# beenotung/bpe-tokenizer

Hardware: NVIDIA B200
Metric: mergeUntil merges/sec (higher is better)
Workload: dtype u32

## Files before the change

### bpe_tokenizer_b200/build.py

```python
from __future__ import annotations

import os
import shutil
import subprocess
import sys

HERE = os.path.dirname(os.path.abspath(__file__))
CSRC = os.path.join(HERE, "csrc")
LIB = os.path.join(HERE, "libbpe_b200.so")
SOURCES = ["bpe_b200.cu", "synth.cpp"]
DEPS = ["common.cuh", "train_kernels.cuh", "encode_kernels.cuh", "encode_lanes.cuh", "encode_dp.cuh", "mg_kernels.cuh", "round_kernels.cuh", "text_kernels.cuh", os.path.join("..", "..", "include", "bpe_b200.h")]
NVCC_FLAGS = [
    "-gencode", "arch=compute_100a,code=sm_100a",
    "-lineinfo", "-O3", "-std=c++17", "-shared",
    "-Xcompiler", "-fPIC,-pthread",
]


def nvcc_path() -> str:
    for cand in (os.environ.get("NVCC"), shutil.which("nvcc"), "/usr/local/cuda/bin/nvcc"):
        if cand and os.path.exists(cand):
            return cand
    raise RuntimeError("nvcc not found")


def needs_build() -> bool:
    if not os.path.exists(LIB):
        return True
    t = os.path.getmtime(LIB)
    return any(os.path.getmtime(os.path.join(CSRC, f)) > t for f in SOURCES + DEPS)


def build(force: bool = False, verbose: bool = False, out: str = LIB) -> str:
    if not force and out == LIB and not needs_build():
        return LIB
    extra = ["-DBPE_FINE_PROF"] if os.environ.get("BPE_FINE_PROF") else []
    if os.environ.get("BPE_ML_THREADS"):
        extra.append("-DBPE_ML_THREADS=" + os.environ["BPE_ML_THREADS"])
    if os.environ.get("BPE_TBL_STRIDE"):
        extra.append("-DBPE_TBL_STRIDE=" + os.environ["BPE_TBL_STRIDE"])
    for knob in ("BPE_R_SMALL_LOG", "BPE_R_BATCH_LOG", "BPE_K1B_CHUNK_LOG"):
        if os.environ.get(knob):
            extra.append("-D%s=%s" % (knob, os.environ[knob]))
    if os.environ.get("BPE_RD_THREADS"):
        extra.append("-DBPE_RD_THREADS=" + os.environ["BPE_RD_THREADS"])
    cmd = [nvcc_path()] + NVCC_FLAGS + extra + (["-Xptxas", "-v"] if verbose else []) + ["-o", out] + [os.path.join(CSRC, f) for f in SOURCES]
    r = subprocess.run(cmd, capture_output=True, text=True)
    if verbose or r.returncode != 0:
        sys.stderr.write(r.stdout + r.stderr)
    if r.returncode != 0:
        raise RuntimeError("nvcc failed (%d)" % r.returncode)
    return out


SYNTH_LIB = os.path.join(HERE, "libbpe_synth.so")


def build_synth(force: bool = False) -> str:
    src = os.path.join(CSRC, "synth.cpp")
    if not force and os.path.exists(SYNTH_LIB) and os.path.getmtime(SYNTH_LIB) >= os.path.getmtime(src):
        return SYNTH_LIB
    cxx = os.environ.get("CXX") or shutil.which("g++") or "g++"
    r = subprocess.run([cxx, "-O2", "-std=c++17", "-shared", "-fPIC", "-pthread", "-o", SYNTH_LIB, src], capture_output=True, text=True)
    if r.returncode != 0:
        sys.stderr.write(r.stdout + r.stderr)
        raise RuntimeError("g++ failed on synth.cpp (%d)" % r.returncode)
    return SYNTH_LIB


if __name__ == "__main__":
    build_synth(force="--force" in sys.argv)
    print(build(force="--force" in sys.argv, verbose="-v" in sys.argv))
```

### bpe_tokenizer_b200/csrc/bpe_b200.cu

```cuda
#include "../../include/bpe_b200.h"

#include <algorithm>
#include <cstdarg>
#include <cstdio>
#include <cstdlib>
#include <chrono>
#include <cstring>
#include <functional>
#include <string>
#include <unordered_map>
#include <vector>

#include "encode_kernels.cuh"
#include "encode_lanes.cuh"
#include "encode_dp.cuh"
#include "train_kernels.cuh"
#include "mg_kernels.cuh"
#include "round_kernels.cuh"
#include "text_kernels.cuh"

using namespace bpe;

namespace {

// ... 934 lines not shown
  if (total > 0) {
    CK(cudaMemsetAsync(&e->d_st.p->err, 0, sizeof(uint32_t), e->stream));
    int blocks = (int)std::min<int64_t>((total / 4 + 255) / 256 + 1, (int64_t)e->grid(8));
    if (reinterpret_cast<const uint32_t*>(dev_ids + base_in) == e->slots.p + e->n_slots)
      k_validate_ids<<<blocks, 256, 0, e->stream>>>(e->slots.p + e->n_slots, (uint64_t)total, (uint32_t)e->n_tokens, &e->d_st.p->err);
    else
      k_ingest_ids<<<blocks, 256, 0, e->stream>>>(dev_ids + base_in, e->slots.p + e->n_slots, (uint64_t)total, (uint32_t)e->n_tokens, &e->d_st.p->err);
    CKL();
    CK(e->stage_off.reserve((size_t)n_docs + 1, 0, e->stream, 1.5));
    CK(cudaMemcpyAsync(e->stage_off.p, host_off, (size_t)(n_docs + 1) * sizeof(int64_t), cudaMemcpyHostToDevice, e->stream));
    int blocks2 = (int)std::min<int64_t>((n_docs + 255) / 256, (int64_t)e->grid(8));
    k_mark_docstarts<<<blocks2, 256, 0, e->stream>>>(e->slots.p, e->stage_off.p, n_docs, (int64_t)e->n_slots - base_in);
    CKL();
    uint32_t bad = 0;
    CK(cudaMemcpyAsync(&bad, &e->d_st.p->err, sizeof bad, cudaMemcpyDeviceToHost, e->stream));
    CK(cudaStreamSynchronize(e->stream));
    if (bad) {
      CK(cudaMemsetAsync(&e->d_st.p->err, 0, sizeof(uint32_t), e->stream));
      return fail(e, BPE_E_INVALID, "document holds a token index >= n_tokens (%d); call bpe_set_tokens first", e->n_tokens);
    }
  }
  for (int64_t d = 0; d < n_docs; d++) e->doc_off.push_back((int64_t)e->n_slots + (host_off[d + 1] - base_in));
  e->n_slots = new_n;
  e->live_tokens += (uint64_t)total;
  e->index_valid = false;
  e->hot_valid = false;
  return BPE_OK;
}


int ensure_round_buffers(bpe_engine* e) {
  if (!e->round_blocks) {
    int per_sm = 0;
    CK(cudaOccupancyMaxActiveBlocksPerMultiprocessor(&per_sm, k_merge_rounds, RD_THREADS, 0));
    if (per_sm < 1) return fail(e, BPE_E_CUDA, "k_merge_rounds does not fit on an SM");
    const int most = std::min({e->sm_count * per_sm, (int)(R_QCAP / RT), RD_THREADS / RT});
    e->round_blocks = std::min(e->sm_count, most);
    if (const char* v = getenv("BPE_LOOP_BLOCKS")) e->round_blocks = std::max(1, std::min(atoi(v), most));
  }
  const size_t cells = (size_t)2 * RB * 2 * ND_STRIDE;
  if (!e->r_cells.p) {
    CK(e->r_cells.reserve(cells));
    CK(cudaMemsetAsync(e->r_cells.p, 0, cells * 8, e->stream));
    CK(e->r_slotrows.reserve(cells));
    CK(e->r_lists.reserve((size_t)2 * e->round_blocks * R_LISTCAP));
    CK(e->r_bsites.reserve((size_t)2 * RB * R_SMALL));
    CK(e->r_state.reserve(1));
    CK(cudaMemsetAsync(e->r_state.p, 0, sizeof(RoundState), e->stream));
  }
  if (e->mg_world > 1 && !e->r_gcells.p) {
    CK(e->r_gcells.reserve(cells));
    CK(cudaMemsetAsync(e->r_gcells.p, 0, cells * 8, e->stream));
    CK(e->r_glists.reserve((size_t)2 * e->round_blocks * R_LISTCAP));
  }
  CK(e->r_gp.reserve((size_t)RT * e->round_blocks));
  CK(e->r_gk.reserve((size_t)RT * e->round_blocks));
  return BPE_OK;
}

RoundArgs round_args(bpe_engine* e, const LoopArgs& L, int round_k) {
  RoundArgs RA{};
  RA.L = L;
  RA.cells = e->r_cells.p;
  RA.slotrows = e->r_slotrows.p;
  RA.lists = e->r_lists.p;
  RA.bsites = e->r_bsites.p;
  RA.gp = e->r_gp.p;
  RA.gk = e->r_gk.p;
  RA.rs = e->r_state.p;
  RA.kmax = (uint32_t)round_k;
  RA.bar_mode = 1;
  if (const char* v = getenv("BPE_LOOP_BAR")) RA.bar_mode = atoi(v) ? 1 : 0;
  RA.mg_on = 0;
  RA.gcells = e->r_gcells.p;
  RA.glists = e->r_glists.p;
  return RA;
}

void round_stats(bpe_engine* e, const RoundState& hrs) {
  e->stats.loop_rounds = (int64_t)hrs.rounds;
  e->stats.loop_round_merges = (int64_t)hrs.round_merges;
  e->stats.loop_round_tried = (int64_t)hrs.tried;
  e->stats.loop_rounds_cut = (int64_t)hrs.rounds_cut_born;
}

int merge_until_device(bpe_engine* e, int64_t min_weight, int32_t max_length, int64_t max_iterations, bpe_merge* log,
                       int64_t log_cap, int64_t* n_done, const int32_t* dev_replay = nullptr) {
  *n_done = 0;
  CK(cudaSetDevice(e->device));
  if (e->n_slots == 0) return BPE_OK;
  TRY(ensure_index(e));
  uint32_t ml = max_length > 0 ? (uint32_t)max_length : 0;
  int64_t mw = min_weight > 0 ? min_weight : 2;
  if (!e->loop_blocks) {
    int per_sm = 0;
    CK(cudaOccupancyMaxActiveBlocksPerMultiprocessor(&per_sm, k_merge_loop, ML_THREADS, 0));
    if (per_sm < 1) return fail(e, BPE_E_CUDA, "k_merge_loop does not fit on an SM");
    int want = 1;
    if (const char* v = getenv("BPE_LOOP_PER_SM")) want = std::max(1, atoi(v));
    e->loop_blocks = e->sm_count * std::min(per_sm, want);
    if (const char* v = getenv("BPE_LOOP_BLOCKS")) e->loop_blocks = std::max(1, std::min(atoi(v), e->sm_count * per_sm));
  }
  bool use_rounds = !dev_replay;
// ... 57 lines not shown
    L.tbl_cap = e->tbl_cap;
    L.sites2 = e->sites2.p;
    L.A.sites_cap = (uint32_t)std::min<size_t>(L.A.sites_cap, e->sites2.cap);
    {
      int a = 12, b = 10, c = 2, ns = 256;
      if (const char* v = getenv("BPE_LOOP_P1_SITES")) a = atoi(v);
      if (const char* v = getenv("BPE_LOOP_P2_NEW")) b = atoi(v);
      if (const char* v = getenv("BPE_LOOP_P2_RW")) c = atoi(v);
      if (const char* v = getenv("BPE_LOOP_BAR_NS")) ns = atoi(v);
      if (a < 1 || a > 15) a = 12;
      if (b < 1 || c < 1 || b + c > 15) b = 10, c = 2;
      L.p1_sites = (uint32_t)a;
      L.p2_new = (uint32_t)b;
      L.p2_rw = (uint32_t)c;
      L.bar_ns = (uint32_t)std::max(32, std::min(ns, 4096));
    }
    const char* pf = getenv("BPE_LOOP_PREFETCH");
    L.prefetch = pf ? std::max(0, std::min(atoi(pf), 2)) : (use_rounds ? 0 : 1);
    L.replay = dev_replay ? dev_replay + 2 * done : nullptr;
    if (dev_replay) e->hot_valid = false;
    static const bool trace = getenv("BPE_TRACE") != nullptr;
    auto tw0 = std::chrono::steady_clock::now();
    k_loop_prepare<<<1, 32, 0, e->stream>>>(e->d_st.p, (uint32_t)e->n_tokens, e->barrier.p);
    e->stats.kernel_launches++;
    if (use_rounds && legacy_above) {
      L.min_weight = (uint32_t)std::max<int64_t>(mw, (int64_t)R_HUGE + 1);
      void* args[] = {&L};
      ce = cudaLaunchCooperativeKernel((void*)k_merge_loop, dim3(e->loop_blocks), dim3(ML_THREADS), args, 0, e->stream);
    } else if (use_rounds) {
      RoundArgs RA = round_args(e, L, round_k);
      k_rounds_prepare<<<1, 32, 0, e->stream>>>(e->r_state.p);
      e->stats.kernel_launches++;
      void* rargs[] = {&RA};
      ce = cudaLaunchCooperativeKernel((void*)k_merge_rounds, dim3(e->round_blocks), dim3(RD_THREADS), rargs, 0, e->stream);
    } else {
      void* args[] = {&L};
      ce = cudaLaunchCooperativeKernel((void*)k_merge_loop, dim3(e->loop_blocks), dim3(ML_THREADS), args, 0, e->stream);
    }
    if (ce != cudaSuccess) {
      rc = fail(e, BPE_E_CUDA, "cooperative launch of the mergeUntil kernel: %s", cudaGetErrorString(ce));
      break;
    }
    e->stats.kernel_launches++;
    if ((rc = fetch_state(e)) != BPE_OK) break;
    uint32_t iters = e->h_st->iters_done;
    if (trace) {
      double ms = std::chrono::duration<double, std::milli>(std::chrono::steady_clock::now() - tw0).count();
      fprintf(stderr, "[bpe] k_merge_loop: %u merges in %.2f ms, status %u, best_cnt %u, hot_n %u thresh %u, keys %u/%u\n", iters, ms,
              e->h_st->status, e->h_st->best_cnt, e->h_st->hot_n, e->h_st->hot_thresh, e->h_st->n_keys, e->tbl_cap);
    }
    if (iters) {
      tmp.resize(iters);
      ce = cudaMemcpyAsync(tmp.data(), e->dev_log.p, (size_t)iters * sizeof(MergeRec), cudaMemcpyDeviceToHost, e->stream);
      if (ce == cudaSuccess) ce = cudaStreamSynchronize(e->stream);
      if (ce != cudaSuccess) {
        rc = fail(e, BPE_E_CUDA, "merge log read-back: %s", cudaGetErrorString(ce));
        break;
      }
      for (uint32_t i = 0; i < iters; i++) {
        const MergeRec& r = tmp[i];
        log[done].a = r.a;
        log[done].b = r.b;
        log[done].c = r.c;
        log[done].reserved = 0;
        log[done].weight = r.weight;
        done++;
        e->h_len16.push_back(e->h_len16[r.a] + e->h_len16[r.b]);
// ... 209 lines not shown
    L.hot = e->hot.p;
    L.hot_cap = (uint32_t)std::min<size_t>(e->hot.cap, 0xFFFFFFF0u);
    L.hot_limit = e->hot_limit;
    L.cands = e->cands.p;
    L.cand_cap = (uint32_t)std::min<size_t>(e->cands.cap, 0xFFFFFFF0u);
    L.partials = e->partials.p;
    L.barrier = e->barrier.p;
    L.log = e->dev_log.p;
    L.log_cap = chunk;
    L.max_length = ml;
    L.min_weight = (uint32_t)std::min<int64_t>(mw, 0xFFFFFFFFll);
    L.max_tokens = BPE_MAX_TOKENS;
    L.tbl_cap = e->tbl_cap;
    L.replay = nullptr;
    P.M = mg_args(e);
    static const bool trace = getenv("BPE_TRACE") != nullptr;
    auto tw0 = std::chrono::steady_clock::now();
    k_loop_prepare<<<1, 32, 0, e->stream>>>(e->d_st.p, (uint32_t)e->n_tokens, e->barrier.p);
    e->stats.kernel_launches++;
    if (use_rounds && !legacy_above) {
      L.sites2 = e->sites2.p;
      L.A.sites_cap = (uint32_t)std::min<size_t>(L.A.sites_cap, e->sites2.cap);
      L.p1_sites = 12;
      L.p2_new = 10;
      L.p2_rw = 2;
      L.bar_ns = 256;
      L.prefetch = 0;
      RoundArgs RA = round_args(e, L, round_k);
      RA.mg_on = 1;
      RA.mg = P.M;
      k_rounds_prepare<<<1, 32, 0, e->stream>>>(e->r_state.p);
      e->stats.kernel_launches++;
      void* rargs[] = {&RA};
      ce = cudaLaunchCooperativeKernel((void*)k_merge_rounds, dim3(e->round_blocks), dim3(RD_THREADS), rargs, 0, e->stream);
    } else {
      if (use_rounds) L.min_weight = (uint32_t)std::max<int64_t>(mw, (int64_t)R_HUGE + 1);
      void* args[] = {&P};
      ce = cudaLaunchCooperativeKernel((void*)k_merge_loop_mg, dim3(e->mg_loop_blocks), dim3(ML_THREADS), args, 0, e->stream);
    }
    if (ce != cudaSuccess) {
      rc = fail(e, BPE_E_CUDA, "cooperative launch of the sharded mergeUntil kernel: %s", cudaGetErrorString(ce));
      break;
    }
    e->stats.kernel_launches++;
    if ((rc = fetch_state(e)) != BPE_OK) break;
    host_ms[2] += since(tw0);
    e->mg_epoch = e->h_st->mg_epoch;
    e->mg_tie_epoch = e->h_st->mg_tie_epoch;
    uint32_t iters = e->h_st->iters_done;
    if (trace) {
      double ms = std::chrono::duration<double, std::milli>(std::chrono::steady_clock::now() - tw0).count();
      fprintf(stderr, "[bpe r%d] k_merge_loop_mg: %u merges in %.2f ms, status %u, best_cnt %u, hot_n %u thresh %u, keys %u/%u err 0x%x gerr 0x%x\n",
              e->mg_rank, iters, ms, e->h_st->status, e->h_st->best_cnt, e->h_st->hot_n, e->h_st->hot_thresh, e->h_st->n_keys, e->tbl_cap,
              e->h_st->err, e->h_st->g_vals[0]);
    }
    auto tl = clk();
    if (iters) {
      tmp.resize(iters);
      ce = cudaMemcpyAsync(tmp.data(), e->dev_log.p, (size_t)iters * sizeof(MergeRec), cudaMemcpyDeviceToHost, e->stream);
      if (ce == cudaSuccess) ce = cudaStreamSynchronize(e->stream);
      if (ce != cudaSuccess) {
        rc = fail(e, BPE_E_CUDA, "merge log read-back: %s", cudaGetErrorString(ce));
        break;
      }
      for (uint32_t i = 0; i < iters; i++) {
        const MergeRec& r = tmp[i];
        log[done].a = r.a;
// ... 1216 lines not shown
```

### bpe_tokenizer_b200/csrc/round_kernels.cuh

```cuda
#pragma once
#include "train_kernels.cuh"
#include "mg_kernels.cuh"

namespace bpe {

#ifndef BPE_RD_THREADS
#define BPE_RD_THREADS 512
#endif
constexpr int RD_THREADS = BPE_RD_THREADS;
constexpr int RB = 16;
#ifndef BPE_R_SMALL_LOG
#define BPE_R_SMALL_LOG 20
#endif
#ifndef BPE_R_BATCH_LOG
#define BPE_R_BATCH_LOG 21
#endif
constexpr uint32_t R_SMALL = 1u << BPE_R_SMALL_LOG;
constexpr uint32_t R_BATCH_SITES = 1u << BPE_R_BATCH_LOG;
constexpr uint32_t R_LAT = 16384;

constexpr uint32_t R_FIELD = 21;
constexpr unsigned long long R_FMASK = (1ull << R_FIELD) - 1ull;
static_assert(BPE_R_SMALL_LOG <= 20, "a batched merge must fit the 21-bit fields of the delta cells (R_HUGE)");
constexpr uint32_t R_HUGE = 1u << 20;
constexpr uint32_t R_POOL_CHUNK = 1u << 16;
constexpr uint32_t R_LISTCAP = 32768;
__host__ __device__ __forceinline__ uint32_t cell_dec(unsigned long long v) { return (uint32_t)(v & R_FMASK); }
__host__ __device__ __forceinline__ uint32_t cell_len(unsigned long long v) { return (uint32_t)((v >> R_FIELD) & R_FMASK); }
__host__ __device__ __forceinline__ uint32_t cell_cnt(unsigned long long v) { return (uint32_t)((v >> (2 * R_FIELD)) & R_FMASK); }
constexpr uint32_t MGR_HDR = 64;
constexpr uint32_t LOOP_NEED_LEGACY = 7;
constexpr uint32_t R_QCAP = 512;

constexpr uint32_t ERR_ROUND_MISMATCH = 2048u;

struct RoundState {
  struct alignas(128) Line {
    uint32_t v;
    uint32_t pad[31];
  };
  struct alignas(128) Line64 {
    unsigned long long v;
    unsigned long long pad[15];
  };
  Line n_sites[2][RB];
  Line64 ub[2][RB];
  uint32_t overflow[2];
  uint32_t goverflow[2];
  uint32_t mg_n[MG_MAX_WORLD];
  unsigned long long mg_ub[RB];
  uint32_t mg_ns[RB];
  uint32_t mg_k;
  uint32_t mg_pad;
  unsigned long long rounds, round_merges, rounds_cut_born, rounds_single, tried;
  unsigned long long stop_reason[8];
  unsigned long long iters_small, iters_big, cells_small, cells_big, sites_small, sites_big;
};

struct RoundArgs {
  LoopArgs L;
  unsigned long long* cells;
  uint32_t* slotrows;
  uint32_t* lists;
  SiteRec* bsites;
  int bar_mode;
  uint4* gp;
  uint32_t* gk;
  RoundState* rs;
  uint32_t kmax;
  int mg_on;
  MgArgs mg;
  unsigned long long* gcells;
  uint32_t* glists;
};

__device__ __forceinline__ unsigned long long* round_cells(const RoundArgs& R, uint32_t par, uint32_t j, uint32_t side) {
  return R.cells + (((size_t)par * RB + j) * 2u + side) * ND_STRIDE;
}
__device__ __forceinline__ uint32_t* round_slotrow(const RoundArgs& R, uint32_t par, uint32_t j, uint32_t side) {
  return R.slotrows + (((size_t)par * RB + j) * 2u + side) * ND_STRIDE;
}
__device__ __forceinline__ uint32_t* round_list(const RoundArgs& R, uint32_t par) {
  return R.lists + ((size_t)par * gridDim.x + blockIdx.x) * R_LISTCAP;
}
__device__ __forceinline__ unsigned long long* round_gcells(const RoundArgs& R, uint32_t par, uint32_t j, uint32_t side) {
  return R.gcells + (((size_t)par * RB + j) * 2u + side) * ND_STRIDE;
}
__device__ __forceinline__ uint32_t* round_glist(const RoundArgs& R, uint32_t par) {
  return R.glists + ((size_t)par * gridDim.x + blockIdx.x) * R_LISTCAP;
}
__device__ __forceinline__ uint32_t round_dec_of(const RoundArgs& R, uint32_t par, uint32_t j, uint32_t side, uint32_t tok) {
  return cell_dec(ld_cg((R.mg_on ? round_gcells(R, par, j, side) : round_cells(R, par, j, side)) + tok));
}

constexpr uint32_t R_NOTOK = 0xFFFFu;
__device__ __forceinline__ uint32_t round_pack_span(uint32_t w, uint32_t p, uint32_t q, uint32_t e) {
  const uint32_t dq = q - p, de = e - p;
  const uint32_t doc = (w & DOCSTART) ? 0x80000000u : 0u;
  if (de >= 32768u) return doc | 0x40000000u;
  return doc | (dq << 15) | de;
}

// ... 70 lines not shown
#pragma unroll
    for (int i = 0; i < RT; i++) {
      w.p[i] = __shfl_xor_sync(0xFFFFFFFFu, v.p[i], o);
      w.s[i] = __shfl_xor_sync(0xFFFFFFFFu, v.s[i], o);
      w.m[i] = __shfl_xor_sync(0xFFFFFFFFu, v.m[i], o);
      w.k[i] = __shfl_xor_sync(0xFFFFFFFFu, v.k[i], o);
    }
#pragma unroll
    for (int i = 0; i < RT; i++) top2_add(v, w.p[i], w.s[i], w.m[i], w.k[i]);
  }
  return v;
}
__device__ __forceinline__ void top2_publish(const Top2& v, uint4* gp, uint32_t* gk, uint32_t bid) {
#pragma unroll
  for (int i = 0; i < RT; i++) {
    gp[RT * bid + i] = make_uint4((uint32_t)v.p[i], (uint32_t)(v.p[i] >> 32), v.s[i], v.m[i]);
    gk[RT * bid + i] = v.k[i];
  }
}

struct RoundSm {
  uint32_t k, status, mult0, pad0;
  uint32_t a[RB], b[RB], w[RB], slot[RB], lstart[RB], llen[RB], lenc[RB];
  uint32_t iter0[RB + 1];
  uint32_t fill_n[RB];
  uint32_t qn;
  unsigned long long qp[R_QCAP];
  uint32_t qs[R_QCAP], qm[R_QCAP], qk[R_QCAP];
  unsigned long long cp[RB];
  uint32_t cs[RB], cm[RB], ck[RB], cls[RB], cll[RB], clen[RB];
  uint32_t g_n_keys, g_pool_cursor, g_snap_err, g_abort;
  uint32_t gv[8];
  uint32_t ncell[2];
  uint32_t gncell[2];
  uint32_t rec_base, rec_cnt;
  uint32_t mg_mask, mg_cnt[MG_MAX_WORLD];
  uint32_t pool_next, pool_end;
  uint32_t keys_ins;
  uint32_t filt_a[8], filt_b[8];
  Top2 t2[32];
  unsigned long long red[32];
  uint32_t s_max[32];
  uint32_t rslot;
};

__device__ __forceinline__ unsigned long long block_max_u64(unsigned long long v, unsigned long long* red) {
#pragma unroll
  for (int o = 16; o > 0; o >>= 1) {
    unsigned long long u = __shfl_xor_sync(0xFFFFFFFFu, v, o);
    v = u > v ? u : v;
  }
  __syncthreads();
  if (lane_id() == 0) red[threadIdx.x >> 5] = v;
  __syncthreads();
  const uint32_t nw = blockDim.x >> 5;
  unsigned long long u = lane_id() < nw ? red[lane_id()] : 0ull;
#pragma unroll
  for (int o = 16; o > 0; o >>= 1) {
    unsigned long long x = __shfl_xor_sync(0xFFFFFFFFu, u, o);
    u = x > u ? x : u;
  }
  return u;
}

__device__ __forceinline__ Top2 top2_block_reduce(Top2 v, Top2* s_t2) {
  v = top2_warp_reduce(v);
  __syncthreads();
  if (lane_id() == 0) s_t2[threadIdx.x >> 5] = v;
  __syncthreads();
  const uint32_t nw = blockDim.x >> 5;
  Top2 u = lane_id() < nw ? s_t2[lane_id()] : top2_empty();
  return top2_warp_reduce(u);
}

__device__ __forceinline__ uint32_t cell_add_warp(const RoundArgs& R, RoundSm& S, uint32_t par, uint32_t js, unsigned long long* cells, uint32_t tok, bool has,
                                                  bool dec, bool newp, bool counted, uint32_t c, uint32_t partner, uint32_t epar) {
  const uint32_t lane = lane_id();
  const uint32_t peers = __match_any_sync(0xFFFFFFFFu, has ? tok : (0xFFFFFF00u + lane));
  const uint32_t dmask = __ballot_sync(0xFFFFFFFFu, has && dec);
  const uint32_t nmask = __ballot_sync(0xFFFFFFFFu, has && newp);
  const uint32_t cmask = __ballot_sync(0xFFFFFFFFu, has && newp && counted);
  const bool leader = has && lane == (uint32_t)(__ffs(peers) - 1);
  uint32_t nc = 0, nd = 0;
  bool first = false;
  if (leader) {
    nc = (uint32_t)__popc(peers & cmask);
    nd = (uint32_t)__popc(peers & dmask);
    const unsigned long long add = (unsigned long long)nd | ((unsigned long long)__popc(peers & nmask) << R_FIELD) | ((unsigned long long)nc << (2 * R_FIELD));
    first = atomicAdd(cells + tok, add) == 0ull;
  }
  const uint32_t fm = __ballot_sync(0xFFFFFFFFu, first);
  if (fm) {
    uint32_t base = 0;
    const int src = __ffs(fm) - 1;
    if ((int)lane == src) base = atomicAdd(&S.ncell[par], (uint32_t)__popc(fm));
    base = __shfl_sync(0xFFFFFFFFu, base, src);
    if (first) {
      const uint32_t k = base + __popc(fm & ((1u << lane) - 1u));
      if (k < R_LISTCAP) round_list(R, par)[k] = (js << 16) | tok;
      else R.rs->overflow[par] = 1;
      const PairTable& t = R.L.A.t;
      const uint32_t side = js & 1u;
      prefetch_l2(t.keys + tbl_hash(t, side ? pair_key(c, tok) : pair_key(tok, c)));
      const uint32_t h2 = tbl_hash(t, side ? pair_key(partner, tok) : pair_key(tok, partner));
      prefetch_l2(t.keys + h2);
      prefetch_l2(t.cnt + h2);
    }
  }
  return nc;
}


__device__ __forceinline__ unsigned long long* mgr_counter(const MgArgs& M, int dst, uint32_t epar, int sender) {
  return M.flag_data[dst] + 16 * sender + 2 + epar;
}

__device__ __forceinline__ void mgr_send_warp(const RoundArgs& R, uint32_t par, uint32_t epar, uint32_t k, unsigned long long epoch, bool with_flag);

__device__ __forceinline__ void round_emit_records(const RoundArgs& R, RoundSm& S, uint32_t par, uint32_t epar, uint32_t k, uint32_t c_hi, unsigned long long epoch) {
  const MgArgs& M = R.mg;
  DevState* st = R.L.A.st;
  const uint32_t cap = M.inbox_stride - MGR_HDR;
  const bool hdr_warp = blockIdx.x == 0 && (threadIdx.x >> 5) == (blockDim.x >> 5) - 1u;
  if (threadIdx.x == 0) S.rec_cnt = 0;
  if (!ld_cg(&R.rs->overflow[par])) {
    const uint32_t n = min(S.ncell[par], R_LISTCAP);
    if (threadIdx.x == 0) {
      S.rec_base = n ? atomicAdd(&st->n_out, n) : 0u;
      S.rec_cnt = n;
    }
    __syncthreads();
    if (hdr_warp) mgr_send_warp(R, par, epar, k, epoch, false);
    const uint32_t base = S.rec_base;
    const uint32_t* list = round_list(R, par);
    for (uint32_t i = threadIdx.x; i < n; i += blockDim.x) {
      const uint32_t ent = ld_cg(list + i);
      const uint32_t js = (ent >> 16) & (2u * RB - 1u), tok = ent & 0xFFFFu;
      const unsigned long long cellv = ld_cg(round_cells(R, par, js >> 1, js & 1u) + tok);
      const unsigned long long rec = ((unsigned long long)ent << 42) | ((unsigned long long)cell_cnt(cellv) << R_FIELD) | cell_dec(cellv);
      const uint32_t at = base + i;
      if (at < cap) {
        for (int q = 0; q < M.world; q++) mg_area(M, q, epar, M.rank)[MGR_HDR + at] = rec;
// ... 187 lines not shown
      const unsigned long long* recs = mg_area(M, M.rank, epar, q) + MGR_HDR;
      uint32_t jx = gtid + G - (uint32_t)q * shift;
      if (jx >= G) jx -= G;
      for (; jx < ((n + 31u) & ~31u); jx += G) {
        bool first = false;
        uint32_t ent = 0;
        if (jx < n) {
          const unsigned long long rec = ld_cg(recs + jx);
          ent = (uint32_t)(rec >> 42);
          const uint32_t js = (ent >> 16) & (2u * RB - 1u), tok = ent & 0xFFFFu;
          first = atomicAdd(round_gcells(R, par, js >> 1, js & 1u) + tok, (rec & ((1ull << (2 * R_FIELD)) - 1ull)) + (1ull << (2 * R_FIELD))) == 0ull;
        }
        const uint32_t fm = __ballot_sync(0xFFFFFFFFu, first);
        if (fm) {
          uint32_t base = 0;
          const int src = __ffs(fm) - 1;
          if ((int)lane == src) base = atomicAdd(&S.gncell[par], (uint32_t)__popc(fm));
          base = __shfl_sync(0xFFFFFFFFu, base, src);
          if (first) {
            const uint32_t at = base + __popc(fm & ((1u << lane) - 1u));
            if (at < R_LISTCAP) round_glist(R, par)[at] = ent;
            else rs->goverflow[par] = 1;
          }
        }
      }
    }
    done |= mask;
    __syncthreads();
  }
  if (warp == 0) mgr_fold_warp(R, epar);
}

__device__ __forceinline__ void round_sites_iter(const RoundArgs& R, RoundSm& S, uint32_t par, uint32_t j, uint32_t c_first,
                                                 uint32_t i, SiteRec* site_out, uint32_t sites_cap, uint32_t epar) {
  const ApplyArgs& A = R.L.A;
  const uint32_t* slots = A.slots;
  const uint32_t n = A.n;
  DevState* st = A.st;
  const uint32_t a = S.a[j], b = S.b[j], c = c_first + j;
  const uint32_t total = S.llen[j];
  const uint32_t lane = lane_id();
  unsigned long long* const cells_l = round_cells(R, par, j, 0);
  unsigned long long* const cells_r = round_cells(R, par, j, 1);
  bool site = false;
  uint32_t p = 0, w = 0, q = 0, koff = 0;
  if (i < total) {
    p = A.pool[S.lstart[j] + i];
    w = ld_slot(slots + p);
    if (slot_is_id(w) && slot_val(w) == a && right_token(slots, n, p, &q) == (int)b) {
      site = true;
      if (a == b) {
        koff = run_left(slots, p, w, (int)a);
        if (koff & 1u) site = false;
      }
    }
  }
  const uint32_t smask = __ballot_sync(0xFFFFFFFFu, site);
  if (!smask) return;
  uint32_t site_base = 0;
  if (lane == (uint32_t)(__ffs(smask) - 1)) site_base = atomicAdd(&R.rs->n_sites[par][j].v, (uint32_t)__popc(smask));
  SiteRec rec{p, NOPOS, R_NOTOK, R_NOTOK};
  uint32_t dec1_tok = 0, new1_tok = 0;
  bool dec1 = false, new1 = false, new1_counted = true;
  if (site) {
    uint32_t lpos;
    int x = left_token(slots, p, w, &lpos);
    if (x != NOTOK) {
      bool chained = false;
      uint32_t chain_j = 0, llpos = NOPOS;
      if (a == b) {
        chained = koff >= 2;
        chain_j = koff >> 1;
        if (chained) left_token(slots, lpos, ld_slot(slots + lpos), &llpos);
// ... 30 lines not shown
          if (S.a[i2] != S.b[i2]) {
            uint32_t l2;
            if (left_token(slots, lpos, wl, &l2) == (int)S.a[i2]) {
              vi = (int)i2;
              vpos = l2;
            }
          } else if (run_left(slots, lpos, wl, x) & 1u) {
            vi = (int)i2;
            left_token(slots, lpos, wl, &vpos);
          }
          break;
        }
        if (vi >= 0) {
          dec1 = true;
          dec1_tok = c_first + (uint32_t)vi;
          new1_tok = c_first + (uint32_t)vi;
          rec.lpos = vpos;
        } else if ((uint32_t)x == a) {
          uint32_t Lr = 1 + run_left(slots, p, w, (int)a);
          dec1 = (Lr & 1u) == 0;
          dec1_tok = a;
          new1_tok = (uint32_t)x;
          rec.lpos = lpos;
        } else {
          dec1 = true;
          dec1_tok = (uint32_t)x;
          new1_tok = (uint32_t)x;
          rec.lpos = lpos;
        }
      }
    }
  }
  const bool dec1_same = dec1 && dec1_tok == new1_tok;
  const uint32_t nc1 = cell_add_warp(R, S, par, j * 2u, cells_l, new1_tok, new1, dec1_same, true, new1_counted, c, a, epar);
  if (__any_sync(0xFFFFFFFFu, dec1 && !dec1_same)) cell_add_warp(R, S, par, j * 2u, cells_l, dec1_tok, dec1 && !dec1_same, true, false, false, c, a, epar);
  rec.lslot = new1 ? new1_tok : R_NOTOK;

  uint32_t dec2_tok = 0, new2_tok = 0, span_word = 0;
  bool dec2 = false, new2 = false;
  if (site) {
    uint32_t r;
    int y = right_token(slots, n, q, &r);
    span_word = round_pack_span(w, p, q, r - 1u);
    if (y != NOTOK) {
      bool chained_right = false;
      if ((uint32_t)y == a) {
        uint32_t r2;
        chained_right = right_token(slots, n, r, &r2) == (int)b;
      }
      if (!chained_right) {
        int vi = -1;
        for (uint32_t i2 = 0; i2 < (role_maybe(S.filt_a, (uint32_t)y) ? j : 0u); i2++) {
          if ((uint32_t)y != S.a[i2]) continue;
          uint32_t r2;
          if (right_token(slots, n, r, &r2) == (int)S.b[i2]) vi = (int)i2;
          break;
        }
        if (vi >= 0) {
          dec2 = true;
          dec2_tok = c_first + (uint32_t)vi;
          new2_tok = c_first + (uint32_t)vi;
        } else if ((uint32_t)y == b && a != b) {
          uint32_t Lr = 1 + run_right(slots, n, q, (int)b);
          dec2 = (Lr & 1u) == 0;
          dec2_tok = b;
          new2_tok = (uint32_t)y;
        } else {
          if (!(a == b && (uint32_t)y == a)) {
            dec2 = true;
            dec2_tok = (uint32_t)y;
          }
          new2_tok = (uint32_t)y;
        }
        new2 = true;
      }
    }
  }
  const bool dec2_same = dec2 && new2 && dec2_tok == new2_tok;
  const uint32_t nc2 = cell_add_warp(R, S, par, j * 2u + 1u, cells_r, new2_tok, new2, dec2_same, true, true, c, b, epar);
  if (__any_sync(0xFFFFFFFFu, dec2 && !dec2_same)) cell_add_warp(R, S, par, j * 2u + 1u, cells_r, dec2_tok, dec2 && !dec2_same, true, false, false, c, b, epar);
  rec.rslot = new2 ? new2_tok : R_NOTOK;
  const uint32_t u1 = __reduce_max_sync(0xFFFFFFFFu, nc1), u2 = __reduce_max_sync(0xFFFFFFFFu, nc2);
  if (lane == 0) {
    if (u1 | u2) atomicAdd(&R.rs->ub[par][j].v, (unsigned long long)u1 | ((unsigned long long)u2 << 32));
  }
  const uint32_t base = __shfl_sync(0xFFFFFFFFu, site_base, __ffs(smask) - 1);
  if (site) {
    const uint32_t k = base + __popc(smask & ((1u << lane) - 1u));
    if (k < sites_cap) reinterpret_cast<uint4*>(site_out)[k] = make_uint4(rec.p, rec.lpos, rec.lslot | (rec.rslot << 16), span_word);
    else atomicOr(&st->err, ERR_SITE_OVERFLOW);
  }
}

__device__ __forceinline__ SiteRec* round_sites_buf(const RoundArgs& R, uint32_t par, uint32_t j) {
  if (j == 0) return par ? R.L.sites2 : R.L.A.sites;
  return R.bsites + ((size_t)par * RB + j) * R_SMALL;
}

struct RoundFill {
  uint32_t v, par, k, c_first;
  uint32_t overflow;
  uint32_t goverflow;
};

__device__ __forceinline__ void round_fill_all(const RoundArgs& R, const RoundSm& S, const RoundFill& F, uint32_t vt, uint32_t nvt) {
  const ApplyArgs& A = R.L.A;
  const PairTable& t = A.t;
  uint32_t total = 0;
  for (uint32_t j = 0; j < F.v; j++) total += (S.fill_n[j] + 31u) & ~31u;
  for (uint32_t i = vt; i < total; i += nvt) {
    uint32_t j = 0, off = i;
    while (off >= ((S.fill_n[j] + 31u) & ~31u)) {
      off -= (S.fill_n[j] + 31u) & ~31u;
// ... 81 lines not shown
  RoundState* rs = R.rs;
  const PairTable& t = A.t;
  const uint32_t bid = blockIdx.x, nblk = gridDim.x;
  const uint32_t tid = threadIdx.x;
  const uint32_t warp = tid >> 5, lane = tid & 31u;
  const uint32_t gt = bid * blockDim.x + tid, gn = nblk * blockDim.x;
  unsigned long long epoch = 0;
  const uint32_t n_tokens0 = ld_cg(&st->n_tokens);
  const uint32_t thresh = ld_cg(&st->hot_thresh);
  const bool lead = (bid == 0 && tid == 0);
#define RBARRIER()                                                        \
  do {                                                                    \
    ++epoch;                                                              \
    if (R.bar_mode) grid_barrier_ra(L.barrier, epoch * nblk, L.bar_ns);   \
    else grid_barrier(L.barrier, epoch * nblk, L.bar_ns);                 \
  } while (0)

  if (lead) st->snap_err = st->err;
  {
    Top2 mine = top2_empty();
    const uint32_t hn = ld_cg(&st->hot_n);
    for (uint32_t i = gt; i < hn; i += gn) {
      const uint32_t hs = L.hot[i];
      uint32_t hk;
      const unsigned long long pr = slot_primary_k(t, A.len16, hs, L.max_length, &hk);
      top2_add(mine, pr, hs, 1, hk);
    }
    const Top2 v = top2_block_reduce(mine, S.t2);
    if (tid == 0) {
      top2_publish(v, R.gp, R.gk, bid);
    }
    if (tid < RB) S.fill_n[tid] = 0;
    if (tid < 2) S.ncell[tid] = S.gncell[tid] = 0;
    if (tid == 0) S.pool_next = S.pool_end = S.keys_ins = 0;
  }
  unsigned long long mg_epoch = R.mg_on ? ld_cg(&st->mg_epoch) : 0ull, tie_epoch = R.mg_on ? ld_cg(&st->mg_tie_epoch) : 0ull;
  unsigned long long mg_prev_alloc = 0;
  if (R.mg_on) {
    if (lead) st->mg_abort = 0;
    if (bid == 0 && warp == 0) mgr_send_warp(R, 0, (uint32_t)((mg_epoch + 1) & 1u), 0, mg_epoch + 1, true);
    if (warp == 0) mgr_wait_fold_warp(R, (uint32_t)((mg_epoch + 1) & 1u), mg_epoch + 1);
    mg_epoch++;
  }
  RBARRIER();

  const bool prof = lead;
  unsigned long long tp0 = prof ? now_ns() : 0, tp1;
  uint32_t prof_big = 0;
#define RPROF(i)                                              \
  if (prof) {                                                 \
    tp1 = now_ns();                                           \
    st->prof_ns[i] += tp1 - tp0;                              \
    if ((i) < 5) st->fine_ns[(prof_big ? 6 : 0) + (i)] += tp1 - tp0; \
    tp0 = tp1;                                                \
  }
  RoundFill F{0, 0, 0, 0, 0, 0};
  uint32_t it = 0;
  for (uint32_t round = 0;; round++) {
    const uint32_t par = round & 1u;
    const uint32_t c_first = n_tokens0 + it;
    const uint32_t hot_pre = ld_cg(&st->hot_n);
    {
      unsigned long long myp = 0;
      uint32_t mys = NOSLOT, mym = 0, myk = 0;
      if (tid < RT * nblk) {
        const uint4 v = ld_cg4(R.gp + tid);
        myp = (unsigned long long)v.x | ((unsigned long long)v.y << 32);
// ... 270 lines not shown
        Best wb{S.cp[0], S.cp[0] ? S.cs[0] : NOSLOT, S.cm[0]};
        publish_best(t, st, wb);
        st->n_cand = 0;
        st->tie_pos = ~0ull;
      }
      return;
    }
    if (F.v && (S.a[0] >= F.c_first || S.b[0] >= F.c_first)) {
      round_fill_all(R, S, F, gt, gn);
      __syncthreads();
      if (tid < RB) S.fill_n[tid] = 0;
      F.v = 0;
      RBARRIER();
    }
    if (bid == 0 && warp == 0) {
      if (lane < k) A.len16[c_first + lane] = S.lenc[lane];
      if (lane < RB) {
        rs->n_sites[par ^ 1u][lane].v = 0;
        rs->ub[par ^ 1u][lane].v = 0;
      }
      if (lane == 0 && S.mult0 > 1) st->tie_breaks++;
    }
    {
      const uint32_t iters = S.iter0[k];
      uint32_t fill_total = 0;
      for (uint32_t j = 0; j < F.v; j++) fill_total += S.fill_n[j];
      const bool split = iters <= 3u * nblk * ((L.p1_sites * (blockDim.x >> 5)) / 16u) && fill_total <= 65536u;
      const uint32_t NW = blockDim.x >> 5;
      const uint32_t ws = split ? (L.p1_sites * NW) / 16u : NW, wh = NW - ws;
      if (warp < ws) {
        for (uint32_t wi = bid * ws + warp; wi < iters; wi += nblk * ws) {
          uint32_t j = 0;
          while (j + 1 < k && wi >= S.iter0[j + 1]) j++;
          round_sites_iter(R, S, par, j, c_first, (wi - S.iter0[j]) * 32u + lane, round_sites_buf(R, par, j), j == 0 ? A.sites_cap : R_SMALL, (uint32_t)((mg_epoch + 1) & 1u));
        }
        if (!split) {
          if (F.v) round_fill_all(R, S, F, gt, gn);
          if (F.k) round_clear_cells(R, S, F, tid, blockDim.x, gt, gn);
        }
      } else {
        const uint32_t hvt = (bid * wh + warp - ws) * 32u + lane, hnvt = nblk * wh * 32u;
        if (F.v) round_fill_all(R, S, F, hvt, hnvt);
        if (F.k) round_clear_cells(R, S, F, (warp - ws) * 32u + lane, wh * 32u, hvt, hnvt);
        if (L.prefetch) {
          uint32_t budget = 32768u;
          for (uint32_t j = k; j < RB && budget; j++) {
            if (!S.cp[j]) break;
            const uint32_t len = min(S.cll[j], budget), start = S.cls[j];
            for (uint32_t i = hvt; i < len; i += hnvt) {
              const uint32_t pp = ld_cg(A.pool + start + i);
              if (pp >= A.n) continue;
              const uint32_t* q = A.slots + pp;
              prefetch_l2(q);
              if (pp >= 12u) prefetch_l2(q - 12);
              if (pp + 28u < A.n) prefetch_l2(q + 28);
            }
            budget -= len;
          }
        }
      }
    }
    RPROF(1)
    RBARRIER();
    RPROF(2)
    if (R.mg_on) {
      const uint32_t epar = (uint32_t)((mg_epoch + 1) & 1u);
      unsigned long long xt0 = prof ? now_ns() : 0, xt1;
#define XPROF(i)                         \
  if (prof) {                            \
    xt1 = now_ns();                      \
    st->mg_prof_ns[5 + (i)] += xt1 - xt0; \
    xt0 = xt1;                           \
  }
      round_emit_records(R, S, par, epar, k, c_first + k, mg_epoch + 1);
      XPROF(0)
      mgr_collect(R, S, par, epar);
      XPROF(1)
      mg_epoch++;
      if (ld_cg(&st->mg_abort)) {
        if (lead) {
          st->status = LOOP_ERROR;
          st->iters_done = it;
          st->n_tokens = n_tokens0 + it;
          st->mg_epoch = mg_epoch;
          st->mg_tie_epoch = tie_epoch;
        }
        return;
      }
      RBARRIER();
      if (bid == 0 && tid < (uint32_t)R.mg.world) {
        *mgr_counter(R.mg, R.mg.rank, epar, (int)tid) = 0ull;
        if (tid == 0) st->n_out = 0;
      }
      XPROF(2)
#undef XPROF
      RPROF(5)
// ... 335 lines not shown
```

Before: 66230.

## Stage hot low-token cell updates in shared memory before flushing to global

For merges with many sites (above a threshold), per-site cell count updates for token ids below a small bound are accumulated with shared-memory atomics in a per-block staging area and flushed to the global cells once per round. The aim is to cut contended global atomics on frequent low-id tokens. In exchange the round kernel needs dynamic shared memory, which may lower occupancy, and it adds a zeroing pass, an extra block sync and a flush loop. The threshold and staging width can be tuned through environment and compile-time settings.

```diff
diff --git a/bpe_tokenizer_b200/build.py b/bpe_tokenizer_b200/build.py
--- a/bpe_tokenizer_b200/build.py
+++ b/bpe_tokenizer_b200/build.py
@@ -39,7 +39,7 @@
         extra.append("-DBPE_ML_THREADS=" + os.environ["BPE_ML_THREADS"])
     if os.environ.get("BPE_TBL_STRIDE"):
         extra.append("-DBPE_TBL_STRIDE=" + os.environ["BPE_TBL_STRIDE"])
-    for knob in ("BPE_R_SMALL_LOG", "BPE_R_BATCH_LOG", "BPE_K1B_CHUNK_LOG"):
+    for knob in ("BPE_R_SMALL_LOG", "BPE_R_BATCH_LOG", "BPE_K1B_CHUNK_LOG", "BPE_STAGE_T"):
         if os.environ.get(knob):
             extra.append("-D%s=%s" % (knob, os.environ[knob]))
     if os.environ.get("BPE_RD_THREADS"):
diff --git a/bpe_tokenizer_b200/csrc/bpe_b200.cu b/bpe_tokenizer_b200/csrc/bpe_b200.cu
--- a/bpe_tokenizer_b200/csrc/bpe_b200.cu
+++ b/bpe_tokenizer_b200/csrc/bpe_b200.cu
@@ -990,7 +990,8 @@
 int ensure_round_buffers(bpe_engine* e) {
   if (!e->round_blocks) {
     int per_sm = 0;
-    CK(cudaOccupancyMaxActiveBlocksPerMultiprocessor(&per_sm, k_merge_rounds, RD_THREADS, 0));
+    CK(cudaFuncSetAttribute(k_merge_rounds, cudaFuncAttributeMaxDynamicSharedMemorySize, (int)R_STAGE_BYTES));
+    CK(cudaOccupancyMaxActiveBlocksPerMultiprocessor(&per_sm, k_merge_rounds, RD_THREADS, R_STAGE_BYTES));
     if (per_sm < 1) return fail(e, BPE_E_CUDA, "k_merge_rounds does not fit on an SM");
     const int most = std::min({e->sm_count * per_sm, (int)(R_QCAP / RT), RD_THREADS / RT});
     e->round_blocks = std::min(e->sm_count, most);
@@ -1027,6 +1028,8 @@
   RA.gk = e->r_gk.p;
   RA.rs = e->r_state.p;
   RA.kmax = (uint32_t)round_k;
+  RA.stage_min = R_STAGE_MIN_DEFAULT;
+  if (const char* v = getenv("BPE_BLOCK_CELLS_MIN_SITES")) RA.stage_min = (uint32_t)std::max(0ll, std::min(atoll(v), 0xFFFFFFFFll));
   RA.bar_mode = 1;
   if (const char* v = getenv("BPE_LOOP_BAR")) RA.bar_mode = atoi(v) ? 1 : 0;
   RA.mg_on = 0;
@@ -1150,7 +1153,7 @@
       k_rounds_prepare<<<1, 32, 0, e->stream>>>(e->r_state.p);
       e->stats.kernel_launches++;
       void* rargs[] = {&RA};
-      ce = cudaLaunchCooperativeKernel((void*)k_merge_rounds, dim3(e->round_blocks), dim3(RD_THREADS), rargs, 0, e->stream);
+      ce = cudaLaunchCooperativeKernel((void*)k_merge_rounds, dim3(e->round_blocks), dim3(RD_THREADS), rargs, R_STAGE_BYTES, e->stream);
     } else {
       void* args[] = {&L};
       ce = cudaLaunchCooperativeKernel((void*)k_merge_loop, dim3(e->loop_blocks), dim3(ML_THREADS), args, 0, e->stream);
@@ -1426,7 +1429,7 @@
       k_rounds_prepare<<<1, 32, 0, e->stream>>>(e->r_state.p);
       e->stats.kernel_launches++;
       void* rargs[] = {&RA};
-      ce = cudaLaunchCooperativeKernel((void*)k_merge_rounds, dim3(e->round_blocks), dim3(RD_THREADS), rargs, 0, e->stream);
+      ce = cudaLaunchCooperativeKernel((void*)k_merge_rounds, dim3(e->round_blocks), dim3(RD_THREADS), rargs, R_STAGE_BYTES, e->stream);
     } else {
       if (use_rounds) L.min_weight = (uint32_t)std::max<int64_t>(mw, (int64_t)R_HUGE + 1);
       void* args[] = {&P};
diff --git a/bpe_tokenizer_b200/csrc/round_kernels.cuh b/bpe_tokenizer_b200/csrc/round_kernels.cuh
--- a/bpe_tokenizer_b200/csrc/round_kernels.cuh
+++ b/bpe_tokenizer_b200/csrc/round_kernels.cuh
@@ -25,6 +25,14 @@
 constexpr uint32_t R_HUGE = 1u << 20;
 constexpr uint32_t R_POOL_CHUNK = 1u << 16;
 constexpr uint32_t R_LISTCAP = 32768;
+#ifndef BPE_STAGE_T
+#define BPE_STAGE_T 256
+#endif
+constexpr uint32_t R_STAGE_T = BPE_STAGE_T;
+constexpr uint32_t R_STAGE_CELLS = RB * 2u * R_STAGE_T;
+constexpr size_t R_STAGE_BYTES = (size_t)R_STAGE_CELLS * (sizeof(unsigned long long) + sizeof(uint16_t));
+static_assert(R_STAGE_CELLS <= 65536u, "a staged cell's index must fit the 16-bit entries of the block's list");
+constexpr uint32_t R_STAGE_MIN_DEFAULT = 16384;
 __host__ __device__ __forceinline__ uint32_t cell_dec(unsigned long long v) { return (uint32_t)(v & R_FMASK); }
 __host__ __device__ __forceinline__ uint32_t cell_len(unsigned long long v) { return (uint32_t)((v >> R_FIELD) & R_FMASK); }
 __host__ __device__ __forceinline__ uint32_t cell_cnt(unsigned long long v) { return (uint32_t)((v >> (2 * R_FIELD)) & R_FMASK); }
@@ -68,6 +76,7 @@
   uint32_t* gk;
   RoundState* rs;
   uint32_t kmax;
+  uint32_t stage_min;
   int mg_on;
   MgArgs mg;
   unsigned long long* gcells;
@@ -204,6 +213,7 @@
   uint32_t g_n_keys, g_pool_cursor, g_snap_err, g_abort;
   uint32_t gv[8];
   uint32_t ncell[2];
+  uint32_t nstage;
   uint32_t gncell[2];
   uint32_t rec_base, rec_cnt;
   uint32_t mg_mask, mg_cnt[MG_MAX_WORLD];
@@ -245,8 +255,33 @@
   return top2_warp_reduce(u);
 }
 
+extern __shared__ __align__(16) unsigned long long r_stage[];
+__device__ __forceinline__ uint16_t* r_stage_list() { return reinterpret_cast<uint16_t*>(r_stage + R_STAGE_CELLS); }
+
+__device__ __forceinline__ void cell_list_first(const RoundArgs& R, RoundSm& S, uint32_t par, uint32_t js, uint32_t tok, bool first, uint32_t c,
+                                                uint32_t partner) {
+  const uint32_t lane = lane_id();
+  const uint32_t fm = __ballot_sync(0xFFFFFFFFu, first);
+  if (!fm) return;
+  uint32_t base = 0;
+  const int src = __ffs(fm) - 1;
+  if ((int)lane == src) base = atomicAdd(&S.ncell[par], (uint32_t)__popc(fm));
+  base = __shfl_sync(0xFFFFFFFFu, base, src);
+  if (first) {
+    const uint32_t k = base + __popc(fm & ((1u << lane) - 1u));
+    if (k < R_LISTCAP) round_list(R, par)[k] = (js << 16) | tok;
+    else R.rs->overflow[par] = 1;
+    const PairTable& t = R.L.A.t;
+    const uint32_t side = js & 1u;
+    prefetch_l2(t.keys + tbl_hash(t, side ? pair_key(c, tok) : pair_key(tok, c)));
+    const uint32_t h2 = tbl_hash(t, side ? pair_key(partner, tok) : pair_key(tok, partner));
+    prefetch_l2(t.keys + h2);
+    prefetch_l2(t.cnt + h2);
+  }
+}
+
 __device__ __forceinline__ uint32_t cell_add_warp(const RoundArgs& R, RoundSm& S, uint32_t par, uint32_t js, unsigned long long* cells, uint32_t tok, bool has,
-                                                  bool dec, bool newp, bool counted, uint32_t c, uint32_t partner, uint32_t epar) {
+                                                  bool dec, bool newp, bool counted, uint32_t c, uint32_t partner, bool staged) {
   const uint32_t lane = lane_id();
   const uint32_t peers = __match_any_sync(0xFFFFFFFFu, has ? tok : (0xFFFFFF00u + lane));
   const uint32_t dmask = __ballot_sync(0xFFFFFFFFu, has && dec);
@@ -259,27 +294,34 @@
     nc = (uint32_t)__popc(peers & cmask);
     nd = (uint32_t)__popc(peers & dmask);
     const unsigned long long add = (unsigned long long)nd | ((unsigned long long)__popc(peers & nmask) << R_FIELD) | ((unsigned long long)nc << (2 * R_FIELD));
-    first = atomicAdd(cells + tok, add) == 0ull;
-  }
-  const uint32_t fm = __ballot_sync(0xFFFFFFFFu, first);
-  if (fm) {
-    uint32_t base = 0;
-    const int src = __ffs(fm) - 1;
-    if ((int)lane == src) base = atomicAdd(&S.ncell[par], (uint32_t)__popc(fm));
-    base = __shfl_sync(0xFFFFFFFFu, base, src);
-    if (first) {
-      const uint32_t k = base + __popc(fm & ((1u << lane) - 1u));
-      if (k < R_LISTCAP) round_list(R, par)[k] = (js << 16) | tok;
-      else R.rs->overflow[par] = 1;
-      const PairTable& t = R.L.A.t;
-      const uint32_t side = js & 1u;
-      prefetch_l2(t.keys + tbl_hash(t, side ? pair_key(c, tok) : pair_key(tok, c)));
-      const uint32_t h2 = tbl_hash(t, side ? pair_key(partner, tok) : pair_key(tok, partner));
-      prefetch_l2(t.keys + h2);
-      prefetch_l2(t.cnt + h2);
-    }
-  }
+    if (staged && tok < R_STAGE_T) {
+      const uint32_t e = js * R_STAGE_T + tok;
+      if (atomicAdd(&r_stage[e], add) == 0ull) r_stage_list()[atomicAdd(&S.nstage, 1u)] = (uint16_t)e;
+    } else {
+      first = atomicAdd(cells + tok, add) == 0ull;
+    }
+  }
+  cell_list_first(R, S, par, js, tok, first, c, partner);
   return nc;
+}
+
+__device__ __forceinline__ void round_flush_stage(const RoundArgs& R, RoundSm& S, uint32_t par, uint32_t c_first) {
+  __syncthreads();
+  const uint32_t ns = S.nstage;
+  const uint16_t* list = r_stage_list();
+  for (uint32_t i0 = threadIdx.x & ~31u; i0 < ns; i0 += blockDim.x) {
+    const uint32_t i = i0 + lane_id();
+    const bool has = i < ns;
+    const uint32_t e = has ? list[i] : 0u;
+    const uint32_t js = e / R_STAGE_T, tok = e - js * R_STAGE_T, j = js >> 1;
+    bool first = false;
+    if (has) {
+      const unsigned long long v = r_stage[e];
+      r_stage[e] = 0ull;
+      first = atomicAdd(round_cells(R, par, j, js & 1u) + tok, v) == 0ull;
+    }
+    cell_list_first(R, S, par, js, tok, first, c_first + j, (js & 1u) ? S.b[j] : S.a[j]);
+  }
 }
 
 
@@ -533,13 +575,14 @@
 }
 
 __device__ __forceinline__ void round_sites_iter(const RoundArgs& R, RoundSm& S, uint32_t par, uint32_t j, uint32_t c_first,
-                                                 uint32_t i, SiteRec* site_out, uint32_t sites_cap, uint32_t epar) {
+                                                 uint32_t i, SiteRec* site_out, uint32_t sites_cap) {
   const ApplyArgs& A = R.L.A;
   const uint32_t* slots = A.slots;
   const uint32_t n = A.n;
   DevState* st = A.st;
   const uint32_t a = S.a[j], b = S.b[j], c = c_first + j;
   const uint32_t total = S.llen[j];
+  const bool staged = total > R.stage_min;
   const uint32_t lane = lane_id();
   unsigned long long* const cells_l = round_cells(R, par, j, 0);
   unsigned long long* const cells_r = round_cells(R, par, j, 1);
@@ -636,8 +679,8 @@
     }
   }
   const bool dec1_same = dec1 && dec1_tok == new1_tok;
-  const uint32_t nc1 = cell_add_warp(R, S, par, j * 2u, cells_l, new1_tok, new1, dec1_same, true, new1_counted, c, a, epar);
-  if (__any_sync(0xFFFFFFFFu, dec1 && !dec1_same)) cell_add_warp(R, S, par, j * 2u, cells_l, dec1_tok, dec1 && !dec1_same, true, false, false, c, a, epar);
+  const uint32_t nc1 = cell_add_warp(R, S, par, j * 2u, cells_l, new1_tok, new1, dec1_same, true, new1_counted, c, a, staged);
+  if (__any_sync(0xFFFFFFFFu, dec1 && !dec1_same)) cell_add_warp(R, S, par, j * 2u, cells_l, dec1_tok, dec1 && !dec1_same, true, false, false, c, a, staged);
   rec.lslot = new1 ? new1_tok : R_NOTOK;
 
   uint32_t dec2_tok = 0, new2_tok = 0, span_word = 0;
@@ -681,8 +724,8 @@
     }
   }
   const bool dec2_same = dec2 && new2 && dec2_tok == new2_tok;
-  const uint32_t nc2 = cell_add_warp(R, S, par, j * 2u + 1u, cells_r, new2_tok, new2, dec2_same, true, true, c, b, epar);
-  if (__any_sync(0xFFFFFFFFu, dec2 && !dec2_same)) cell_add_warp(R, S, par, j * 2u + 1u, cells_r, dec2_tok, dec2 && !dec2_same, true, false, false, c, b, epar);
+  const uint32_t nc2 = cell_add_warp(R, S, par, j * 2u + 1u, cells_r, new2_tok, new2, dec2_same, true, true, c, b, staged);
+  if (__any_sync(0xFFFFFFFFu, dec2 && !dec2_same)) cell_add_warp(R, S, par, j * 2u + 1u, cells_r, dec2_tok, dec2 && !dec2_same, true, false, false, c, b, staged);
   rec.rslot = new2 ? new2_tok : R_NOTOK;
   const uint32_t u1 = __reduce_max_sync(0xFFFFFFFFu, nc1), u2 = __reduce_max_sync(0xFFFFFFFFu, nc2);
   if (lane == 0) {
@@ -830,7 +873,8 @@
     }
     if (tid < RB) S.fill_n[tid] = 0;
     if (tid < 2) S.ncell[tid] = S.gncell[tid] = 0;
-    if (tid == 0) S.pool_next = S.pool_end = S.keys_ins = 0;
+    if (tid == 0) S.pool_next = S.pool_end = S.keys_ins = S.nstage = 0;
+    for (uint32_t i = tid; i < R_STAGE_CELLS; i += blockDim.x) r_stage[i] = 0ull;
   }
   unsigned long long mg_epoch = R.mg_on ? ld_cg(&st->mg_epoch) : 0ull, tie_epoch = R.mg_on ? ld_cg(&st->mg_tie_epoch) : 0ull;
   unsigned long long mg_prev_alloc = 0;
@@ -1167,7 +1211,7 @@
         for (uint32_t wi = bid * ws + warp; wi < iters; wi += nblk * ws) {
           uint32_t j = 0;
           while (j + 1 < k && wi >= S.iter0[j + 1]) j++;
-          round_sites_iter(R, S, par, j, c_first, (wi - S.iter0[j]) * 32u + lane, round_sites_buf(R, par, j), j == 0 ? A.sites_cap : R_SMALL, (uint32_t)((mg_epoch + 1) & 1u));
+          round_sites_iter(R, S, par, j, c_first, (wi - S.iter0[j]) * 32u + lane, round_sites_buf(R, par, j), j == 0 ? A.sites_cap : R_SMALL);
         }
         if (!split) {
           if (F.v) round_fill_all(R, S, F, gt, gn);
@@ -1194,9 +1238,13 @@
           }
         }
       }
+      bool staging = false;
+      for (uint32_t j = 0; j < k; j++) staging |= S.llen[j] > R.stage_min;
+      if (staging) round_flush_stage(R, S, par, c_first);
     }
     RPROF(1)
     RBARRIER();
+    if (tid == 0) S.nstage = 0;
     RPROF(2)
     if (R.mg_on) {
       const uint32_t epar = (uint32_t)((mg_epoch + 1) & 1u);
```

Result: faster. 68980, median of 6 (+4.2%).
